# xiph/daala

Measured on AMD Instinct MI355X. Metric: 1080p all-intra transform blocks/s (filter+DCT+PVQ), higher is better.
Workload: dtype int32 (lifting DCT/filters) + f64 (PVQ search)

## Files before the change

daala_amd/csrc/od_occupancy.cuh:

```cuda
#pragma once
#ifndef ODHIP_SEARCH_OCC
# define ODHIP_SEARCH_OCC 0
#endif
#if ODHIP_SEARCH_OCC == 2
# define OD_SEARCH_OCC_ATTR __attribute__((amdgpu_waves_per_eu(2), amdgpu_num_vgpr(100)))
# define OD_SEARCH_VGPR_FLOOR() asm volatile("" ::: "v175")
#elif ODHIP_SEARCH_OCC == 3
# define OD_SEARCH_OCC_ATTR __attribute__((amdgpu_waves_per_eu(3), amdgpu_num_vgpr(68)))
# define OD_SEARCH_VGPR_FLOOR() asm volatile("" ::: "v128")
#else
# define OD_SEARCH_OCC_ATTR __attribute__((amdgpu_waves_per_eu(3)))
# define OD_DECIDE_OCC_ATTR
# define OD_SEARCH_VGPR_FLOOR() ((void)0)
#endif
#ifndef OD_DECIDE_OCC_ATTR
# define OD_DECIDE_OCC_ATTR OD_SEARCH_OCC_ATTR
#endif
#ifndef ODHIP_SEARCH_WAVES
# define ODHIP_SEARCH_WAVES 1
#endif
#ifndef ODHIP_PAIR_WAVES
# define ODHIP_PAIR_WAVES 8
#endif
#ifndef OD_PAIR_OCC_ATTR
# if ODHIP_SEARCH_OCC == 0
#  define OD_PAIR_OCC_ATTR __attribute__((amdgpu_waves_per_eu(4)))
# else
#  define OD_PAIR_OCC_ATTR OD_SEARCH_OCC_ATTR
# endif
#endif
```

daala_amd/csrc/pvq_refbands.hip:

```cpp
#include "../../include/daala_hip.h"
#include <math.h>
#include <stdio.h>
#include <stdlib.h>
#include <string.h>
#include "od_ctx.cuh"
#include "od_pvq_math.cuh"
#include "od_occupancy.cuh"
#include "od_krange.cuh"
#include "od_band_stage.cuh"
#include "gen/od_scan_tables.h"
#define OD_RSQ_TABLE_N 512
#define OD_RSQ_HUGE
#include "pvq_search.cuh"
#include "pvq_row.cuh"
#include "pvq_regs.cuh"
#include "pvq_lane.cuh"

namespace {

constexpr int kMaxJobs = 8;
constexpr int kMaxItems = kMaxJobs*ODHIP_MAX_BANDS;
constexpr int kSlots = ODHIP_PVQ_REF_SLOTS;
constexpr int kUncCap = 1 << 16;
constexpr double kDefaultMargin = 1e-9;
// ... 1246 lines not shown
      cos_out[band] = c;
      if (replays_out) replays_out[band] = replays;
    }
  }
  (void)n;
}

template <int E, int G>
__global__ __launch_bounds__(kWave) __attribute__((amdgpu_waves_per_eu(3, 3))) void k_refb_search_row(RItems it) {
  od_rsqrt_init(threadIdx.x);
  const int item = find_item(it, blockIdx.x);
  const RJob &jb = it.jobs[it.job[item]];
  const int lane = threadIdx.x;
  RowVector<E, G> v;
  v.row = lane/G;
  v.l = lane%G;
  v.force = it.perturb >> 1;
  const long nblocks = jb.nblocks;
  const long pos = (long)(blockIdx.x - it.wg_start[item])*(kWave/G) + v.row;
  const bool live = pos < nblocks;
  const long blk = jb.ids[(long)it.band[item]*nblocks + (live ? pos : nblocks - 1)];
  NoDecide nd;
  refb_loops(jb, it.band[item], blk, live && v.l == 0, live, it.lambda, v, nd);
}

template <int N>
struct RegVector {
  static constexpr int SH = N == 15 ? 1 : 0;
  int ax[N];
  unsigned sg;
  int y[N];
  double xx;
  double norm_1;
  double cxy;
  double cyy;
  __device__ __forceinline__ void load(const int16_t *src, bool pad) {
    const uint4 *p = reinterpret_cast<const uint4 *>(src - SH);
    sg = 0;
    uint32_t w[(N + SH)/2];
#pragma unroll
    for (int q = 0; q < (N + SH)/8; q++) {
      const uint4 t = p[q];
      w[4*q] = t.x;
      w[4*q + 1] = t.y;
      w[4*q + 2] = t.z;
      w[4*q + 3] = t.w;
    }
#pragma unroll
    for (int i = 0; i < N; i++) {
      const int t = (int16_t)(w[(i + SH) >> 1] >> (16*((i + SH) & 1)));
      ax[i] = abs(t);
      sg |= (unsigned)(t < 0) << i;
      y[i] = 0;
    }
    if (pad) {
      ax[N - 1] = 0;
      sg &= ~(1u << (N - 1));
    }
    od_regs_norm<N>(ax, &xx, &norm_1);
  }
  __device__ __forceinline__ double search(int n_true, int k, int prev_k, double g2, double lambda) {
    return od_pvq_search_regs<N>(ax, y, n_true, k, prev_k, g2, lambda, xx, norm_1, &cxy, &cyy);
  }
  __device__ __forceinline__ int moment() const {
    int m = 0;
#pragma unroll
    for (int i = 1; i < N; i++) m += i*y[i];
    return m;
  }
  __device__ __forceinline__ void store(int16_t *dst) {
    uint4 *p = reinterpret_cast<uint4 *>(dst - SH);
    int t[N + SH];
    if (SH) t[0] = 0;
#pragma unroll
    for (int i = 0; i < N; i++) t[i + SH] = (sg >> i) & 1 ? -y[i] : y[i];
#pragma unroll
    for (int q = 0; q < (N + SH)/8; q++) {
      p[q] = make_uint4(pack16(t[8*q], t[8*q + 1]), pack16(t[8*q + 2], t[8*q + 3]),
       pack16(t[8*q + 4], t[8*q + 5]), pack16(t[8*q + 6], t[8*q + 7]));
    }
  }
};

template <int NL>
struct PairVector {
  struct Pulses {
    const uint32_t *col;
    __device__ __forceinline__ int operator[](int e) const { return (int)(col[e*kPitch] >> 1 & 0x7fffu); }
  };
  uint32_t *pk;
  Pulses y;
  unsigned sg;
  int lane;
  int l;
  bool force_seq;
  LaneSearch st;
  __device__ __forceinline__ void init(uint32_t *columns, int lane_in, bool force) {
    pk = columns;
    y.col = columns + lane_in;
    lane = lane_in;
    l = lane_in & 1;
    force_seq = force;
  }
  __device__ __forceinline__ void load(const int16_t *src, bool pad) {
    static_assert(NL % 8 == 0, "whole 16-byte pieces");
    const uint4 *p = reinterpret_cast<const uint4 *>(src + l*NL);
    sg = 0;
#pragma unroll
    for (int q = 0; q < NL/8; q++) {
      const uint4 t = p[q];
      const uint32_t w[4] = {t.x, t.y, t.z, t.w};
#pragma unroll
      for (int e = 0; e < 8; e++) {
        const int j = 8*q + e;
        int v = (int16_t)(w[e >> 1] >> (16*(e & 1)));
        if (j == NL - 1 && pad && l == 1) v = 0;
        pk[j*kPitch + lane] = (uint32_t)abs(v) << 16;
        sg |= (unsigned)(v < 0) << j;
      }
    }
    od_lane_prepare<NL, 2>(st, pk, lane);
  }
  __device__ __forceinline__ double search(int n_true, int k, int prev_k, double g2, double lambda) {
    const bool fresh = !(prev_k > 0 && prev_k <= k);
    return od_lane_search<NL, 2, true>(st, pk, od_rsq_lds, lane, l, true, fresh, k, g2, lambda, force_seq,
     n_true != 2*NL);
  }
  __device__ __forceinline__ int moment() const {
    int m = 0;
#pragma unroll
    for (int e = 0; e < NL; e++) m += (l*NL + e)*y[e];
    return od_grp_add<2>(m);
  }
};

__device__ __forceinline__ int neg_interleave(int x, int ref) {
  if (x < ref) return -2*(x - ref) - 1;
  if (x < 2*ref) return 2*(x - ref);
  return x - 1;
}

__device__ unsigned char gRBandOf[OD_SCAN_LEN];

template <int N, class YGet>
__device__ __forceinline__ void refb_finish(const RItems &it, int job, const RJob &jb, int band, long blk,
 const odhip_pvq_refband &r, const RefBest &best, YGet yget);

template <int N, int PRICE>
__device__ __forceinline__ void refb_choose_band(const RItems &it, int job, const RJob &jb, int band,
 long blk, const double *given) {
  constexpr int SH = N == 15 ? 1 : 0;
  constexpr int NW = (N + SH)/2;
  const long bi = blk*jb.nb_bands + band;
  const odhip_pvq_refband r = jb.rec[bi];
  const ItemPtr ip = item_ptr(jb, band, blk);
  const double *rate = PRICE == 2 ? given : PRICE == 0 && jb.rate ? jb.rate + bi*(kSlots + 1) : nullptr;
  const double lambda = it.lambda;
  const int off = jb.off[band];
  double best_cost = r.dist0 + lambda*(rate ? rate[0] : 0.);
  bool close = false;
  int noref = jb.is_keyframe ? 1 : 0;
  int32_t best_qtheta = 0;
  int chosen = -1;
  int yslot = -1;
  int4 tails[kSlots];
  int dlo[kSlots];
  int dhi[kSlots];
#pragma unroll
  for (int idx = 0; idx < kSlots; idx++) {
    tails[idx] = make_int4(0, 0, 0, -1);
    dlo[idx] = 0;
    dhi[idx] = 0;
    if (idx < r.nitems) {
      tails[idx] = ip.tail[idx*ip.stride];
      const int4 res = ip.res[idx*ip.stride];
      dlo[idx] = res.z;
      dhi[idx] = res.w;
    }
  }
#pragma unroll
  for (int idx = 0; idx < kSlots; idx++) {
    if (idx >= r.nitems) continue;
    const int4 tail = tails[idx];
    if (!(tail.z & ODHIP_REFITEM_SEARCHED)) continue;
    double cost = __hiloint2double(dhi[idx], dlo[idx]);
    if (PRICE == 1) {
      const int4 hd = ip.head[idx*ip.stride];
      const bool with_ref = idx < r.ntheta;
      const int sum = (int)((unsigned)tail.z >> ODHIP_REFITEM_MOMENT_SHIFT);
      cost = cost + lambda*odq_pvq_rate_fast(sum, hd.w, N, hd.x, with_ref ? r.icgr : 0, with_ref ? hd.y : -1,
       with_ref ? hd.z : 0, jb.is_keyframe, jb.pli);
      const double d = cost - best_cost;
      if ((d < 0 ? -d : d) <= it.tol_scale*odq_rate_tol(cost, best_cost)) close = true;
    }
    else cost = cost + lambda*(rate ? rate[1 + idx] : 0.);
    if (idx < r.ntheta ? cost < best_cost : cost <= best_cost) {
      best_cost = cost;
      chosen = idx;
      yslot = tail.w;
      if (idx < r.ntheta) {
        best_qtheta = tail.y;
        noref = 0;
      }
      else noref = 1;
    }
  }
  RefBest best;
  best.best_cost = best_cost;
  best.chosen = chosen;
  best.yslot = yslot;
  best.noref = noref;
  best.qtheta = best_qtheta;
  best.gain = best.theta = best.ts = best.k = 0;
  best.close = PRICE == 1 && close;
  if (chosen >= 0) {
    const int4 head = ip.head[chosen*ip.stride];
    best.gain = head.x;
// ... 384 lines not shown
      dist = (1.4*(qcg - cg))*(qcg - cg) + (qcg*(double)cg)*dist_theta;
      dist *= s2;
      const double lts = __hiloint2double((int)cl.col[(kSlots + 7 + 2*gi)*cl.stride],
       (int)cl.col[(kSlots + 6 + 2*gi)*cl.stride]);
      dec.offer(idx - 1, true, i, j, ts, k, qtheta, dist, prate, lts, has, v);
    }
  }
  if (cl.nitems > cl.ntheta) {
    v.load(jb.x16 + blk*len + off, false);
    int prev_k = 0;
    int idx = cl.ntheta;
    while (idx < cl.nitems) {
      const uint32_t w = cl.col[idx*cl.stride];
      const int i = cl.gbn + (int)(w & 3u);
#ifdef ODHIP_EXPERIMENTS
      const int k = dec.abl & 8 ? 0 : (int)(w >> 2 & 0xffffu);
#else
      const int k = (int)(w >> 2 & 0xffffu);
#endif
      const int32_t qcg = odq_shl32(i, ODQ_CGAIN_SHIFT);
      double dist = (1.4*(qcg - cg))*(qcg - cg);
      dist *= s2;
      const bool skip = (dist > dist0 && k != 0) || k > ODHIP_PVQ_MAX_K;
      const bool others = __any(skip);
      if (!skip && others) continue;
      idx++;
      if (skip) continue;
      const double cos_dist = v.search(n, k, prev_k, (qcg*(double)cg)*s2, lambda);
      prev_k = k;
      const double prate = lean_rate_pulses<NR>(v.moment(), k);
      dist = (1.4*(qcg - cg))*(qcg - cg) + (qcg*(double)cg)*(2 - 2*cos_dist);
      dist *= s2;
      dec.offer(idx - 1, false, i, -1, 0, k, 0, dist, prate, 0., true, v);
    }
  }
}

constexpr int kPreWords = 6;
constexpr int kPrePacked = 1;

template <int NR, int G, class V, class D, bool PACKED = false, int WAVES = kSearchWaves>
__device__ __forceinline__ void refb_loops_lean_rows(const RJob &jb, int band, long blk,
 const odhip_pvq_refband &r, const CandList &cl, double lambda, V &v, D &dec, uint32_t *pre, int pre_stride) {
  const int off = jb.off[band];
  const int n = jb.off[band + 1] - off;
  const int len = jb.len;
  const double s2 = (1./256)*(1./256);
  const double t1 = 1./32768;
  const int32_t cg = r.cg;
  const double dist0 = r.dist0;
  const int32_t theta = r.theta;
  uint32_t skips = 0;
  for (int c = v.l; c < kSlots; c += G) {
    if (c < cl.ntheta) {
      const uint32_t w = cl.col[c*cl.stride];
      const int gi = (int)(w & 3u);
      const int k = (int)(w >> 2 & 0xffffu);
      const int i = cl.gb1 + gi;
      const int ts = (int)cl.col[(kSlots + gi)*cl.stride];
      const int j = (int)cl.col[(kSlots + 3 + gi)*cl.stride] + (int)(w >> 18);
      const int32_t qcg = odq_shl32(i, ODQ_CGAIN_SHIFT) + r.gain_offset;
      const int32_t qtheta = odq_pvq_compute_theta(j, ts);
      const int cosd = odq_pvq_cos(theta - qtheta);
      const double cosfix = 2 - (2.*cosd)*t1;
      double dist = (1.4*(qcg - cg))*(qcg - cg) + (qcg*(double)cg)*cosfix;
      dist *= s2;
      const bool skip = (dist > dist0 + 1.0*lambda && k != 0) || k > ODHIP_PVQ_MAX_K;
      if constexpr (PACKED) {
        skips |= (uint32_t)skip << c;
        pre[c*kPrePacked*pre_stride] = ((uint32_t)cosd & 0xffffu) | (uint32_t)odq_pvq_sin(qtheta) << 16;
      }
      else {
        const double sin_prod = ((odq_pvq_sin(theta)*t1)*odq_pvq_sin(qtheta))*t1;
        uint32_t *p = pre + c*kPreWords*pre_stride;
        p[0] = (uint32_t)qcg;
        p[pre_stride] = skip;
        p[2*pre_stride] = (uint32_t)__double2loint(cosfix);
        p[3*pre_stride] = (uint32_t)__double2hiint(cosfix);
        p[4*pre_stride] = (uint32_t)__double2loint(sin_prod);
        p[5*pre_stride] = (uint32_t)__double2hiint(sin_prod);
      }
    }
  }
  static_assert(!PACKED || (G == 2 && kSlots <= 32), "the two halves of a pair's skip mask");
  if constexpr (PACKED) skips = od_grp_or<2>(skips);
  if constexpr (WAVES == 1) __syncthreads();
  else {
    __builtin_amdgcn_fence(__ATOMIC_RELEASE, "wavefront");
    __builtin_amdgcn_wave_barrier();
    __builtin_amdgcn_fence(__ATOMIC_ACQUIRE, "wavefront");
  }
  if (cl.ntheta > 0) {
    v.load(jb.xr + blk*len + off, true);
    int prev_k = 0;
    bool has = false;
    double cos_dist = 0;
    double prate = 0;
    int idx = 0;
    while (idx < cl.ntheta) {
      const uint32_t w = cl.col[idx*cl.stride];
#ifdef ODHIP_EXPERIMENTS
      const int k = dec.abl & 8 ? 0 : (int)(w >> 2 & 0xffffu);
#else
      const int k = (int)(w >> 2 & 0xffffu);
#endif
      const uint32_t *p = pre + idx*(PACKED ? kPrePacked : kPreWords)*pre_stride;
      const bool skip = PACKED ? (skips >> idx & 1u) != 0 : p[pre_stride] != 0;
      const bool want = !skip && k != 0 && k != prev_k;
      const bool others = __any(!want);
      if (want && others) continue;
      idx++;
      if (skip) continue;
      const int gi = (int)(w & 3u);
      const int i = cl.gb1 + gi;
      const int ts = (int)cl.col[(kSlots + gi)*cl.stride];
      const int j = (int)cl.col[(kSlots + 3 + gi)*cl.stride] + (int)(w >> 18);
      int32_t qcg;
      double cosfix;
      double sin_prod;
      if constexpr (PACKED) {
        const uint32_t cs = p[0];
        qcg = odq_shl32(i, ODQ_CGAIN_SHIFT) + r.gain_offset;
        cosfix = 2 - (2.*(int16_t)(cs & 0xffffu))*t1;
        sin_prod = ((odq_pvq_sin(theta)*t1)*(int16_t)(cs >> 16))*t1;
      }
      else {
        qcg = (int32_t)p[0];
        cosfix = __hiloint2double((int)p[3*pre_stride], (int)p[2*pre_stride]);
        sin_prod = __hiloint2double((int)p[5*pre_stride], (int)p[4*pre_stride]);
      }
      if (k == 0) {
        cos_dist = 0;
        has = false;
        prate = 0;
      }
      else if (want) {
        cos_dist = v.search(n - 1, k, prev_k, ((qcg*(double)cg)*sin_prod)*s2, lambda);
        has = true;
        prate = lean_rate_pulses<NR>(v.moment(), k);
      }
      prev_k = k;
      const double dist_theta = cosfix + sin_prod*(2 - 2*cos_dist);
      double dist = (1.4*(qcg - cg))*(qcg - cg) + (qcg*(double)cg)*dist_theta;
      dist *= s2;
      const double lts = __hiloint2double((int)cl.col[(kSlots + 7 + 2*gi)*cl.stride],
       (int)cl.col[(kSlots + 6 + 2*gi)*cl.stride]);
      dec.offer(idx - 1, true, i, j, ts, k, 0, dist, prate, lts, has, v);
    }
  }
  if (cl.nitems > cl.ntheta) {
    v.load(jb.x16 + blk*len + off, false);
    int prev_k = 0;
    int idx = cl.ntheta;
    while (idx < cl.nitems) {
      const uint32_t w = cl.col[idx*cl.stride];
      const int i = cl.gbn + (int)(w & 3u);
#ifdef ODHIP_EXPERIMENTS
      const int k = dec.abl & 8 ? 0 : (int)(w >> 2 & 0xffffu);
#else
      const int k = (int)(w >> 2 & 0xffffu);
#endif
      const int32_t qcg = odq_shl32(i, ODQ_CGAIN_SHIFT);
      double dist = (1.4*(qcg - cg))*(qcg - cg);
      dist *= s2;
      const bool skip = (dist > dist0 && k != 0) || k > ODHIP_PVQ_MAX_K;
      const bool others = __any(skip);
      if (!skip && others) continue;
      idx++;
      if (skip) continue;
      const double cos_dist = v.search(n, k, prev_k, (qcg*(double)cg)*s2, lambda);
      prev_k = k;
      const double prate = lean_rate_pulses<NR>(v.moment(), k);
      dist = (1.4*(qcg - cg))*(qcg - cg) + (qcg*(double)cg)*(2 - 2*cos_dist);
      dist *= s2;
      dec.offer(idx - 1, false, i, -1, 0, k, 0, dist, prate, 0., true, v);
    }
  }
}

template <int NY>
struct LeanDecide {
  double best_cost;
  int chosen;
  bool close;
  int y[NY];
  unsigned sg;
  double lambda;
  double tol_scale;
  int icgr;
  int is_keyframe;
  int pli;
#ifdef ODHIP_EXPERIMENTS
  int abl = 0;
#endif
  __device__ __forceinline__ void init(const odhip_pvq_refband &r, const RJob &jb, double lam, double tol) {
    best_cost = r.dist0;
    chosen = -1;
    close = false;
    lambda = lam;
    tol_scale = tol;
    icgr = r.icgr;
    is_keyframe = jb.is_keyframe;
    pli = jb.pli;
    sg = 0;
#pragma unroll
    for (int i = 0; i < NY; i++) y[i] = 0;
  }
  template <class V>
  __device__ __forceinline__ void offer(int idx, bool with_ref, int i, int j, int ts, int k, int32_t qtheta,
   double dist, double prate, double lts, bool has, const V &v) {
    const double rate = odq_pvq_rate_join(prate, lts, i, with_ref ? icgr : 0, with_ref ? j : -1, is_keyframe,
     pli);
    const double cost = dist + lambda*rate;
    const double d = cost - best_cost;
    if ((d < 0 ? -d : d) <= tol_scale*odq_rate_tol(cost, best_cost)) close = true;
    if (with_ref ? cost < best_cost : cost <= best_cost) {
      best_cost = cost;
      chosen = idx;
      sg = v.sg;
#pragma unroll
      for (int e = 0; e < NY; e++) y[e] = has ? v.y[e] : 0;
    }
    (void)ts;
    (void)k;
    (void)qtheta;
  }
  __device__ __forceinline__ int signed_y(int e) const {
    return (sg >> e) & 1 ? -y[e] : y[e];
  }
};

template <int NY>
__device__ __forceinline__ RefBest lean_best(const LeanDecide<NY> &dec, const CandList &cl, int is_keyframe) {
  RefBest b;
  b.best_cost = dec.best_cost;
  b.chosen = dec.chosen;
  b.yslot = -1;
  b.noref = is_keyframe ? 1 : 0;
  b.qtheta = 0;
  b.gain = b.theta = b.ts = b.k = 0;
  b.close = dec.close;
  if (dec.chosen >= 0) {
    const uint32_t w = cl.col[dec.chosen*cl.stride];
    b.k = (int)(w >> 2 & 0xffffu);
    b.yslot = b.k > 0 ? 0 : -1;
    if (dec.chosen < cl.ntheta) {
      const int gi = (int)(w & 3u);
      b.noref = 0;
      b.gain = cl.gb1 + gi;
      b.ts = (int)cl.col[(kSlots + gi)*cl.stride];
      b.theta = (int)cl.col[(kSlots + 3 + gi)*cl.stride] + (int)(w >> 18);
      b.qtheta = odq_pvq_compute_theta(b.theta, b.ts);
    }
    else {
      b.noref = 1;
      b.gain = cl.gbn + (int)(w & 3u);
    }
  }
  return b;
}

template <int N>
__global__ __launch_bounds__(kSearchThreads) OD_SEARCH_OCC_ATTR void k_refb_lean_lane(RItems it) {
  constexpr int SH = N == 15 ? 1 : 0;
  __shared__ uint32_t s_list_w[kSearchWaves][kLeanWords*kWave];
  OD_SEARCH_VGPR_FLOOR();
  od_rsqrt_init(threadIdx.x);
  const int lane = threadIdx.x%kWave;
  const int wave = __builtin_amdgcn_readfirstlane(threadIdx.x/kWave);
// ... 138 lines not shown
    return;
  }
  const int m = r.m;
  const int s = r.s;
  scale = (int32_t)floor(.5 + (scale*(1./32768))*odq_pvq_sin(best.qtheta));
  const int16_t xm = (int16_t)floor(.5 + ((-s*odq_shr_round(g, gshift))*(1./32768))*odq_pvq_cos(best.qtheta));
  uint32_t rw[E/2];
#pragma unroll
  for (int q = 0; q < E/8; q++) {
    const uint4 r4 = reinterpret_cast<const uint4 *>(jb.r16 + blk*jb.len + off + l*E)[q];
    rw[4*q] = r4.x;
    rw[4*q + 1] = r4.y;
    rw[4*q + 2] = r4.z;
    rw[4*q + 3] = r4.w;
  }
  const int yprev = grp_from_prev<G>(wy[E - 1], l);
  int32_t l2r = 0;
  int32_t proj = 0;
#pragma unroll
  for (int e = 0; e < E; e++) {
    const int i = l*E + e;
    const int ri = (int16_t)(rw[e >> 1] >> (16*(e & 1)));
    const int ysrc = i < m ? wy[e] : (e == 0 ? yprev : wy[e > 0 ? e - 1 : 0]);
    const int16_t xi = i == m ? xm : (int16_t)odq_mult16_32_q16(ysrc, scale);
    l2r += odq_mult16_16(ri, ri);
    proj += odq_mult16_16(ri, xi);
  }
  l2r = grp_total<G>(l2r);
  proj = grp_total<G>(proj);
  int16_t proj_1;
  int outshift;
  householder_consts(l2r, proj, &proj_1, &outshift);
  if (writer) {
    ch[2] = make_int4(3, yslot, scale, qshift);
    ch[3] = make_int4(xm, m, proj_1, outshift);
  }
  (void)n;
}

template <int E, int G>
__global__ __launch_bounds__(kSearchThreads) OD_SEARCH_OCC_ATTR void k_refb_lean_row(RItems it) {
  constexpr int C = kWave/G;
  __shared__ uint32_t s_list_w[kSearchWaves][kLeanWords*C];
  __shared__ uint32_t s_pre_w[kSearchWaves][kSlots*kPreWords*C];
  OD_SEARCH_VGPR_FLOOR();
  od_rsqrt_init(threadIdx.x);
  const int wave = __builtin_amdgcn_readfirstlane(threadIdx.x/kWave);
  const int unit = blockIdx.x*kSearchWaves + wave;
  if (unit >= it.wg_start[it.nitems]) return;
  uint32_t *s_list = s_list_w[wave];
  uint32_t *s_pre = s_pre_w[wave];
  const int item = find_item(it, unit);
  const int job = it.job[item];
  const RJob &jb = it.jobs[job];
  const int band = it.band[item];
  const int lane = threadIdx.x%kWave;
  RowVector<E, G> v;
  v.row = lane/G;
  v.l = lane%G;
  v.force = it.perturb >> 1;
  const long nblocks = jb.nblocks;
  const long pos = (long)(unit - it.wg_start[item])*C + v.row;
  const bool live = pos < nblocks;
  const long blk = jb.ids[(long)band*nblocks + (live ? pos : nblocks - 1)];
  const odhip_pvq_refband r = jb.rec[blk*jb.nb_bands + band];
  const CandList cl = refb_build_list(jb, band, r, s_list + v.row, C, v.l == 0);
  LeanDecide<E> dec;
  dec.init(r, jb, it.lambda, it.tol_scale);
#ifdef ODHIP_EXPERIMENTS
  dec.abl = it.abl;
#endif
  refb_loops_lean_rows<G*E, G>(jb, band, blk, r, cl, it.lambda, v, dec, s_pre + v.row, C);
  refb_finish_row<E, G>(it, job, jb, band, blk, r, dec, lean_best(dec, cl, jb.is_keyframe), v.l, live);
#ifdef ODHIP_EXPERIMENTS
  if (live && v.l == 0) {
    if (v.pulses) atomicAdd(&gRowReplayStats[0], (unsigned long long)v.pulses);
    if (v.replays) atomicAdd(&gRowReplayStats[1], (unsigned long long)v.replays);
    if (v.rate_pulses) atomicAdd(&gRowReplayStats[2], (unsigned long long)v.rate_pulses);
    atomicAdd(&gRowReplayStats[3], 1ull);
  }
#endif
}

constexpr int kPairWaves = ODHIP_PAIR_WAVES;
constexpr int kPairThreads = kPairWaves*kWave;

template <int NL>
__global__ __launch_bounds__(kPairThreads) OD_PAIR_OCC_ATTR void k_refb_lean_pair(RItems it) {
  constexpr int G = 2;
  constexpr int C = kWave/G;
  static_assert(kRsqN == OD_RSQ_TABLE_N && kPitch == kWave, "od_lane_search on this unit's table and columns");
  __shared__ uint32_t s_list_w[kPairWaves][kLeanWords*C];
  __shared__ uint32_t s_pre_w[kPairWaves][kSlots*kPrePacked*C];
  __shared__ uint32_t s_pk_w[kPairWaves][NL*kPitch];
  OD_SEARCH_VGPR_FLOOR();
  od_rsqrt_init(threadIdx.x);
  const int wave = __builtin_amdgcn_readfirstlane(threadIdx.x/kWave);
  const int unit = blockIdx.x*kPairWaves + wave;
  if (unit >= it.wg_start[it.nitems]) return;
  uint32_t *s_list = s_list_w[wave];
  uint32_t *s_pre = s_pre_w[wave];
  const int item = find_item(it, unit);
  const int job = it.job[item];
  const RJob &jb = it.jobs[job];
  const int band = it.band[item];
  const int lane = threadIdx.x%kWave;
  const int row = lane/G;
  PairVector<NL> v;
  v.init(s_pk_w[wave], lane, (it.perturb >> 1) != 0);
  const long nblocks = jb.nblocks;
  const long pos = (long)(unit - it.wg_start[item])*C + row;
  const bool live = pos < nblocks;
  const long blk = jb.ids[(long)band*nblocks + (live ? pos : nblocks - 1)];
  const odhip_pvq_refband r = jb.rec[blk*jb.nb_bands + band];
  const CandList cl = refb_build_list(jb, band, r, s_list + row, C, v.l == 0);
  LeanDecide<NL> dec;
  dec.init(r, jb, it.lambda, it.tol_scale);
#ifdef ODHIP_EXPERIMENTS
  dec.abl = it.abl;
#endif
  refb_loops_lean_rows<G*NL, G, PairVector<NL>, LeanDecide<NL>, true, kPairWaves>(jb, band, blk, r, cl,
   it.lambda, v, dec, s_pre + row, C);
  refb_finish_row<NL, G>(it, job, jb, band, blk, r, dec, lean_best(dec, cl, jb.is_keyframe), v.l, live);
}

template <int N>
__global__ __launch_bounds__(kWave) void k_refb_choose_unc_list(RItems it, const Unc *list, int count) {
  const int i = blockIdx.x*kWave + threadIdx.x;
  if (i >= count) return;
  const Unc e = list[i];
  const RJob &jb = it.jobs[e.job];
  if (jb.off[e.band + 1] - jb.off[e.band] != N) return;
  refb_choose_band<N, 1>(it, e.job, jb, e.band, e.blk, nullptr);
}

template <int N, int PRICE>
__global__ __launch_bounds__(kWave) void k_refb_choose(RItems it) {
  const int item = find_item(it, blockIdx.x);
  const int job = it.job[item];
  const RJob &jb = it.jobs[job];
  const long blk = (long)(blockIdx.x - it.wg_start[item])*kWave + threadIdx.x;
  if (blk >= jb.nblocks) return;
  refb_choose_band<N, PRICE>(it, job, jb, it.band[item], blk, nullptr);
}

template <int N>
__global__ __launch_bounds__(kWave) void k_refb_choose_list(RItems it, const PUncR *list, int count) {
  const int i = blockIdx.x*kWave + threadIdx.x;
  if (i >= count) return;
  const PUncR *e = list + i;
  const RJob &jb = it.jobs[e->job];
  if (jb.off[e->band + 1] - jb.off[e->band] != N) return;
  refb_choose_band<N, 2>(it, e->job, jb, e->band, e->blk, e->rate);
}

__global__ __launch_bounds__(256) void k_refb_synth(RItems it) {
  const int item = find_item(it, blockIdx.x);
  const RJob &jb = it.jobs[it.job[item]];
  const int len = jb.len;
  const int cpb = len >> 3;
  const long t = (long)(blockIdx.x - it.wg_start[item])*256 + threadIdx.x;
  const long blk = t/cpb;
  if (blk >= jb.nblocks) return;
  const int c0 = (int)(t - blk*cpb) << 3;
  const long base = block_base(jb, blk);
  od_coeff *out = jb.dq + base;
  const int w = jb.w;
  const int band = gRBandOf[c0 ? c0 : 1];
  const int off = jb.off[band];
  const uint4 sc4 = *reinterpret_cast<const uint4 *>(gRScanPk + c0);
  const unsigned scw[4] = {sc4.x, sc4.y, sc4.z, sc4.w};
  long pos[8];
#pragma unroll
  for (int e = 0; e < 8; e++) {
    const unsigned pk = (scw[e >> 1] >> (16*(e & 1))) & 0xffffu;
    pos[e] = (long)(pk >> 8)*w + (pk & 255);
  }
  const int4 *ch = reinterpret_cast<const int4 *>(jb.choice + (blk*jb.nb_bands + band)*16);
  const int4 a = ch[2];
  const int mode = a.x;
  const int first = c0 == 0;
  if (first) out[0] = jb.coef[base];
  if (mode == 0) {
#pragma unroll
    for (int e = 0; e < 8; e++) if (!(first && e == 0)) out[pos[e]] = 0;
    return;
  }
  if (mode == 1 || mode == 4) {
#pragma unroll
    for (int e = 0; e < 8; e++) {
      if (first && e == 0) continue;
      const od_coeff rv = jb.ref[base + pos[e]];
      out[pos[e]] = mode == 4 ? -rv : rv;
    }
    return;
  }
  const int yslot = a.y;
  const int32_t scale = a.z;
  const int qshift = a.w;
  const uint4 q4 = *reinterpret_cast<const uint4 *>(jb.qm_inv + c0);
  const unsigned qw[4] = {q4.x, q4.y, q4.z, q4.w};
  unsigned yw[4] = {0, 0, 0, 0};
  int yprev = 0;
  if (yslot >= 0) {
// ... 202 lines not shown
  for (int i = 0; i < njobs; i++) {
    rc = fill_job(host[i], jobs[i], mode);
    if (rc) return rc;
    host[i].krange = st.counters.d.p + 2;
  }
  if (mode == kJobBands) {
    rc = st.sort.place(host, njobs, s);
    if (rc) return rc;
  }
  return st.tabs.upload(host, njobs, s);
}

int sort_weights(void) {
  static const int w = [] {
    int p = 4, c = 4, s = 8;
    const char *e = ODHIP_EXP_ENV("ODHIP_SORT_W");
    if (e) sscanf(e, "%d,%d,%d", &p, &c, &s);
    return (p & 255) | (c & 255) << 8 | (s & 255) << 16;
  }();
  return w;
}

void items_begin(RItems &it, const RefState &st, double lambda) {
  memset(&it, 0, sizeof(it));
  it.lambda = lambda;
  it.margin = st.margin;
  it.perturb = st.perturb;
  it.jobs = st.tabs.cur;
  it.unc_count = st.unc_count();
  it.unc = st.unc.p;
  it.pcount = st.pcount();
  it.plist = st.plist.p;
  it.tol_scale = st.tol_scale;
  it.sort_weights = sort_weights();
#ifdef ODHIP_EXPERIMENTS
  static const int abl = [] {
    const char *e = getenv("ODHIP_REFB_ABL");
    return e ? atoi(e) : 0;
  }();
  it.abl = abl;
#endif
}

enum RefStage {
  kStageRecords = 0,
  kStageLanePriced = 1,
  kStageDecided = 2
};

void launch_prep(const RefState &st, const RJob *host, int njobs, double lambda, RefStage stage, hipStream_t s) {
  RItems pi;
  const auto prep = [&](void (*kernel)(RItems), int size, long per_wg) {
    items_begin(pi, st, lambda);
    pi.fuse = stage;
    if (size) items_add_size(pi, host, njobs, size, per_wg, 1);
    else for (int j = 0; j < njobs; j++) items_add(pi, j, 0, (host[j].nblocks + per_wg - 1)/per_wg);
    if (pi.nitems) kernel<<<pi.wg_start[pi.nitems], kWave, 0, s>>>(pi);
  };
#ifdef ODHIP_EXPERIMENTS
  static const bool split = getenv("ODHIP_REFB_PREP_SPLIT") != nullptr;
  if (split) {
    prep(k_refb_prep_lane<15>, 0, kWave);
    prep(k_refb_prep_lane<8>, 8, kWave);
  }
  else
#endif
  prep(k_refb_prep_corner, 0, kWave);
  prep(k_refb_prep_row<8, 4>, 32, 16);
  prep(k_refb_prep_row<8, 16>, 128, 4);
}

int sort_blocks(RefState &st, const RJob *host, int njobs, hipStream_t s) {
  return st.sort.run(host, st.tabs.cur, njobs, s);
}

struct RefSearch {
  int size;
  int on;
  int per_wg;
  bool row;
};
constexpr RefSearch kRefSearches[4] = {{128, 0, 4, true}, {32, 1, 16, true}, {15, 2, kWave, false},
 {8, 2, kWave, false}};
constexpr int kPairBands = kWave/2;

bool pair_search(const RefSearch &r, RefStage stage) {
  static const bool row32 = ODHIP_EXP_ENV("ODHIP_REFB_ROW32") != nullptr;
  return r.size == 32 && stage == kStageDecided && !row32;
}

void launch_search(RefState &st, RItems &it, const RefSearch &r, RefStage stage, hipStream_t s) {
  if (stage == kStageDecided) items_heavy_first(it);
  const int wgs = it.wg_start[it.nitems];
  const int groups = (wgs + kSearchWaves - 1)/kSearchWaves;
  const auto regs = [&](auto priced) {
    for_band_size(r.size, [&](auto size) {
      constexpr int N = decltype(size)::value;
      if constexpr (N <= 15) k_refb_search_regs<N, decltype(priced)::value><<<wgs, kWave, 0, s>>>(it);
    });
  };
  const auto launch = [&] {
    if (pair_search(r, stage)) k_refb_lean_pair<16><<<(wgs + kPairWaves - 1)/kPairWaves, kPairThreads, 0, s>>>(it);
    else if (r.row) {
      for_band_size(r.size, [&](auto size) {
        constexpr int N = decltype(size)::value;
        if constexpr (N >= 32) {
          if (stage == kStageDecided) k_refb_lean_row<8, N/8><<<groups, kSearchThreads, 0, s>>>(it);
          else k_refb_search_row<8, N/8><<<wgs, kWave, 0, s>>>(it);
        }
      });
    }
    else if (stage == kStageDecided) {
      for_band_size(r.size, [&](auto size) {
        constexpr int N = decltype(size)::value;
        if constexpr (N <= 15) k_refb_lean_lane<N><<<groups, kSearchThreads, 0, s>>>(it);
      });
    }
    else if (stage == kStageLanePriced) regs(std::true_type());
    else regs(std::false_type());
  };
  if (r.size == 128) st.prof.around(s, launch);
  else launch();
}

int launch_searches(RefState &st, const RJob *host, int njobs, double lambda, RefStage stage, hipStream_t s) {
  const bool lane_only = stage != kStageDecided && ODHIP_EXP_ENV("ODHIP_PVQ_REF_LANE") != nullptr;
  hipStream_t side[2] = {s, s};
  if (st.streams.fork(s, side) != ODHIP_SUCCESS) return ODHIP_EFAULT;
  const hipStream_t streams[3] = {s, side[0], side[1]};
  RItems it;
  for (const RefSearch &r : kRefSearches) {
    items_begin(it, st, lambda);
    if (r.row && !lane_only && odhip_env_force_seq()) it.perturb |= 2;
    items_add_size(it, host, njobs, r.size, lane_only ? kWave : pair_search(r, stage) ? kPairBands : r.per_wg);
    if (it.nitems && !lane_only) launch_search(st, it, r, stage, streams[r.on]);
#ifdef ODHIP_EXPERIMENTS
    if (it.nitems && lane_only) {
      k_refb_search<<<it.wg_start[it.nitems], kWave, (size_t)2*r.size*kWave*sizeof(unsigned short), streams[r.on]>>>(it);
    }
#endif
  }
  if (st.streams.join(s, side) != ODHIP_SUCCESS) return ODHIP_EFAULT;
  return ODHIP_SUCCESS;
}

int ref_bands(const odhip_pvq_refjob *jobs, int njobs, double pvq_norm_lambda, odhip_stream stream, RefStage stage) {
  hipStream_t s = (hipStream_t)stream;
  REF_STATE_OR_RETURN(st);
  RJob host[kMaxJobs];
  int rc = stage_jobs(st, jobs, njobs, kJobBands, host, s);
  if (rc) return rc;
  ODHIP_TRY(hipMemsetAsync(st.unc_count(), 0, (stage != kStageRecords ? 2 : 1)*sizeof(unsigned), s));
  st.lean = stage == kStageDecided;
  RItems it;
  items_begin(it, st, pvq_norm_lambda);
  items_add_size(it, host, njobs, 0, kWave);
  if (!it.nitems) return ODHIP_SUCCESS;
  launch_prep(st, host, njobs, pvq_norm_lambda, stage, s);
  if (stage != kStageDecided) k_refb_cands<<<it.wg_start[it.nitems], kWave, 0, s>>>(it);
  rc = sort_blocks(st, host, njobs, s);
  if (rc) return rc;
  rc = launch_searches(st, host, njobs, pvq_norm_lambda, stage, s);
  if (rc) return rc;
  if (stage == kStageDecided) {
    rc = st.unc_posted.post(st.unc_count(), s);
    if (!rc) rc = st.priced.post(st.pcount(), s);
    if (rc) return rc;
  }
  return odhip_check_launch();
}

void rerun_listed(const RefState &st, const Unc *d_list, unsigned n, double lambda, hipStream_t s) {
  k_refb_cands_list<<<(n + kWave - 1)/kWave, kWave, 0, s>>>(st.tabs.cur, d_list, (int)n);
  k_refb_search_list<<<n, kWave, (size_t)2*128*kWave*sizeof(unsigned short), s>>>(st.tabs.cur, d_list, (int)n,
   lambda);
}

void decide_listed(RefState &st, const Unc *d_list, unsigned n, double lambda, hipStream_t s) {
  RItems it;
  items_begin(it, st, lambda);
  const unsigned grid = (n + kWave - 1)/kWave;
  for (const int size : kBandSizes) {
    for_band_size(size, [&](auto N) {
      k_refb_choose_unc_list<decltype(N)::value><<<grid, kWave, 0, s>>>(it, d_list, (int)n);
    });
  }
  (void)st.priced.post(st.pcount(), s);
}

enum RefSelect {
  kSelectSynth,
  kSelectChoice,
  kSelectPriced,
  kSelectPricedRest
};

int ref_select(const odhip_pvq_refjob *jobs, int njobs, double pvq_norm_lambda, hipStream_t s, RefSelect sel) {
  const bool synth = sel == kSelectSynth;
  const bool price = sel == kSelectPriced || sel == kSelectPricedRest;
  REF_STATE_OR_RETURN(st);
  RJob host[kMaxJobs];
  int rc = stage_jobs(st, jobs, njobs, synth ? kJobSynth : kJobChoice, host, s);
  if (rc) return rc;
  for (int j = 0; synth && j < njobs; j++) {
    if (host[j].bs >= 3) {
      const size_t bytes = sizeof(od_coeff)*(size_t)host[j].nplanes*host[j].w*host[j].h;
      if (host[j].is_keyframe) ODHIP_TRY(hipMemsetAsync(host[j].dq, 0, bytes, s));
      else ODHIP_TRY(hipMemcpyAsync(host[j].dq, host[j].ref, bytes, hipMemcpyDeviceToDevice, s));
    }
  }
  if (sel == kSelectPriced) ODHIP_TRY(hipMemsetAsync(st.pcount(), 0, sizeof(unsigned), s));
  RItems it;
  const auto choose = [&](int n, auto priced) {
    for_band_size(n, [&](auto N) {
      k_refb_choose<decltype(N)::value, decltype(priced)::value><<<it.wg_start[it.nitems], kWave, 0, s>>>(it);
    });
  };
// ... 234 lines not shown
```

Measured before the change: 1.232 billion.

## Search 128-coefficient bands with lane groups in the decided PVQ stage

Generalizes the pair-lane lean search kernel into a GroupVector kernel, where S lanes share one band and each lane holds NL coefficients. In the decided stage, 128-coefficient bands now run through this kernel with four lanes per band (32 coefficients each) instead of the row kernel that packs 4 bands per workgroup. The goal is to fit 16 bands into each wave and cut the per-band serial work, at the cost of more LDS per wave, 64-bit sign masks, and different occupancy and wave-count settings.

```diff
diff --git a/daala_amd/csrc/od_occupancy.cuh b/daala_amd/csrc/od_occupancy.cuh
--- a/daala_amd/csrc/od_occupancy.cuh
+++ b/daala_amd/csrc/od_occupancy.cuh
@@ -22,10 +22,29 @@
 #ifndef ODHIP_PAIR_WAVES
 # define ODHIP_PAIR_WAVES 8
 #endif
-#ifndef OD_PAIR_OCC_ATTR
+#ifndef ODHIP_PAIR_OCC
+# define ODHIP_PAIR_OCC 4
+#endif
+#ifndef ODHIP_GROUP128_LANES
+# define ODHIP_GROUP128_LANES 4
+#endif
+#ifndef ODHIP_GROUP128_WAVES
+# define ODHIP_GROUP128_WAVES 4
+#endif
+#ifndef ODHIP_GROUP128_OCC
+# define ODHIP_GROUP128_OCC 3
+#endif
+#ifndef ODHIP_GROUP128_PAIR_WAVES
+# define ODHIP_GROUP128_PAIR_WAVES 6
+#endif
+#ifndef ODHIP_GROUP128_PAIR_OCC
+# define ODHIP_GROUP128_PAIR_OCC 2
+#endif
+#ifndef OD_GROUP_OCC_ATTR
 # if ODHIP_SEARCH_OCC == 0
-#  define OD_PAIR_OCC_ATTR __attribute__((amdgpu_waves_per_eu(4)))
+#  define OD_GROUP_OCC_ATTR(nl, s) __attribute__((amdgpu_waves_per_eu( \
+    (nl)*(s) == 32 ? ODHIP_PAIR_OCC : (s) == 4 ? ODHIP_GROUP128_OCC : ODHIP_GROUP128_PAIR_OCC)))
 # else
-#  define OD_PAIR_OCC_ATTR OD_SEARCH_OCC_ATTR
+#  define OD_GROUP_OCC_ATTR(nl, s) OD_SEARCH_OCC_ATTR
 # endif
 #endif
diff --git a/daala_amd/csrc/pvq_refbands.hip b/daala_amd/csrc/pvq_refbands.hip
--- a/daala_amd/csrc/pvq_refbands.hip
+++ b/daala_amd/csrc/pvq_refbands.hip
@@ -1352,15 +1352,22 @@
   }
 };
 
-template <int NL>
-struct PairVector {
+template <int NY>
+struct LeanSigns {
+  using type = std::conditional_t<(NY > 32), unsigned long long, unsigned>;
+};
+
+template <int NL, int S>
+struct GroupVector {
+  static_assert(S == 2 || S == 4, "a pair or a quad per band");
   struct Pulses {
     const uint32_t *col;
     __device__ __forceinline__ int operator[](int e) const { return (int)(col[e*kPitch] >> 1 & 0x7fffu); }
   };
+  using Signs = typename LeanSigns<NL>::type;
   uint32_t *pk;
   Pulses y;
-  unsigned sg;
+  Signs sg;
   int lane;
   int l;
   bool force_seq;
@@ -1369,7 +1376,7 @@
     pk = columns;
     y.col = columns + lane_in;
     lane = lane_in;
-    l = lane_in & 1;
+    l = lane_in & (S - 1);
     force_seq = force;
   }
   __device__ __forceinline__ void load(const int16_t *src, bool pad) {
@@ -1384,25 +1391,27 @@
       for (int e = 0; e < 8; e++) {
         const int j = 8*q + e;
         int v = (int16_t)(w[e >> 1] >> (16*(e & 1)));
-        if (j == NL - 1 && pad && l == 1) v = 0;
+        if (j == NL - 1 && pad && l == S - 1) v = 0;
         pk[j*kPitch + lane] = (uint32_t)abs(v) << 16;
-        sg |= (unsigned)(v < 0) << j;
+        sg |= (Signs)(v < 0) << j;
       }
     }
-    od_lane_prepare<NL, 2>(st, pk, lane);
+    od_lane_prepare<NL, S>(st, pk, lane);
   }
   __device__ __forceinline__ double search(int n_true, int k, int prev_k, double g2, double lambda) {
     const bool fresh = !(prev_k > 0 && prev_k <= k);
-    return od_lane_search<NL, 2, true>(st, pk, od_rsq_lds, lane, l, true, fresh, k, g2, lambda, force_seq,
-     n_true != 2*NL);
+    return od_lane_search<NL, S, true>(st, pk, od_rsq_lds, lane, l, true, fresh, k, g2, lambda, force_seq,
+     n_true != S*NL);
   }
   __device__ __forceinline__ int moment() const {
     int m = 0;
 #pragma unroll
     for (int e = 0; e < NL; e++) m += (l*NL + e)*y[e];
-    return od_grp_add<2>(m);
+    return od_grp_add<S>(m);
   }
 };
+template <int NL>
+using PairVector = GroupVector<NL, 2>;
 
 __device__ __forceinline__ int neg_interleave(int x, int ref) {
   if (x < ref) return -2*(x - ref) - 1;
@@ -1953,8 +1962,8 @@
       }
     }
   }
-  static_assert(!PACKED || (G == 2 && kSlots <= 32), "the two halves of a pair's skip mask");
-  if constexpr (PACKED) skips = od_grp_or<2>(skips);
+  static_assert(!PACKED || ((G == 2 || G == 4) && kSlots <= 32), "the parts of a group's skip mask");
+  if constexpr (PACKED) skips = od_grp_or<G>(skips);
   if constexpr (WAVES == 1) __syncthreads();
   else {
     __builtin_amdgcn_fence(__ATOMIC_RELEASE, "wavefront");
@@ -2055,7 +2064,7 @@
   int chosen;
   bool close;
   int y[NY];
-  unsigned sg;
+  typename LeanSigns<NY>::type sg;
   double lambda;
   double tol_scale;
   int icgr;
@@ -2360,21 +2369,25 @@
 #endif
 }
 
-constexpr int kPairWaves = ODHIP_PAIR_WAVES;
-constexpr int kPairThreads = kPairWaves*kWave;
-
-template <int NL>
-__global__ __launch_bounds__(kPairThreads) OD_PAIR_OCC_ATTR void k_refb_lean_pair(RItems it) {
-  constexpr int G = 2;
+constexpr int kGroup128Lanes = ODHIP_GROUP128_LANES;
+static_assert(kGroup128Lanes == 4 || kGroup128Lanes == 2, "a quad or a pair per 128-coefficient band");
+
+template <int NL, int S>
+constexpr int kGroupWaves = NL*S == 32 ? ODHIP_PAIR_WAVES : S == 4 ? ODHIP_GROUP128_WAVES : ODHIP_GROUP128_PAIR_WAVES;
+
+template <int NL, int S>
+__global__ __launch_bounds__((kGroupWaves<NL, S>*kWave)) OD_GROUP_OCC_ATTR(NL, S) void k_refb_lean_pair(RItems it) {
+  constexpr int G = S;
+  constexpr int WAVES = kGroupWaves<NL, S>;
   constexpr int C = kWave/G;
   static_assert(kRsqN == OD_RSQ_TABLE_N && kPitch == kWave, "od_lane_search on this unit's table and columns");
-  __shared__ uint32_t s_list_w[kPairWaves][kLeanWords*C];
-  __shared__ uint32_t s_pre_w[kPairWaves][kSlots*kPrePacked*C];
-  __shared__ uint32_t s_pk_w[kPairWaves][NL*kPitch];
+  __shared__ uint32_t s_list_w[WAVES][kLeanWords*C];
+  __shared__ uint32_t s_pre_w[WAVES][kSlots*kPrePacked*C];
+  __shared__ uint32_t s_pk_w[WAVES][NL*kPitch];
   OD_SEARCH_VGPR_FLOOR();
   od_rsqrt_init(threadIdx.x);
   const int wave = __builtin_amdgcn_readfirstlane(threadIdx.x/kWave);
-  const int unit = blockIdx.x*kPairWaves + wave;
+  const int unit = blockIdx.x*WAVES + wave;
   if (unit >= it.wg_start[it.nitems]) return;
   uint32_t *s_list = s_list_w[wave];
   uint32_t *s_pre = s_pre_w[wave];
@@ -2384,7 +2397,7 @@
   const int band = it.band[item];
   const int lane = threadIdx.x%kWave;
   const int row = lane/G;
-  PairVector<NL> v;
+  GroupVector<NL, S> v;
   v.init(s_pk_w[wave], lane, (it.perturb >> 1) != 0);
   const long nblocks = jb.nblocks;
   const long pos = (long)(unit - it.wg_start[item])*C + row;
@@ -2397,7 +2410,7 @@
 #ifdef ODHIP_EXPERIMENTS
   dec.abl = it.abl;
 #endif
-  refb_loops_lean_rows<G*NL, G, PairVector<NL>, LeanDecide<NL>, true, kPairWaves>(jb, band, blk, r, cl,
+  refb_loops_lean_rows<G*NL, G, GroupVector<NL, S>, LeanDecide<NL>, true, WAVES>(jb, band, blk, r, cl,
    it.lambda, v, dec, s_pre + row, C);
   refb_finish_row<NL, G>(it, job, jb, band, blk, r, dec, lean_best(dec, cl, jb.is_keyframe), v.l, live);
 }
@@ -2766,11 +2779,26 @@
 };
 constexpr RefSearch kRefSearches[4] = {{128, 0, 4, true}, {32, 1, 16, true}, {15, 2, kWave, false},
  {8, 2, kWave, false}};
-constexpr int kPairBands = kWave/2;
-
-bool pair_search(const RefSearch &r, RefStage stage) {
-  static const bool row32 = ODHIP_EXP_ENV("ODHIP_REFB_ROW32") != nullptr;
-  return r.size == 32 && stage == kStageDecided && !row32;
+
+int group_lanes(const RefSearch &r, RefStage stage) {
+  if (stage != kStageDecided) return 0;
+  if (r.size == 32) {
+    static const bool row32 = ODHIP_EXP_ENV("ODHIP_REFB_ROW32") != nullptr;
+    return row32 ? 0 : 2;
+  }
+  if (r.size == 128) {
+#ifdef ODHIP_EXPERIMENTS
+    static const int lanes = [] {
+      const char *e = ODHIP_EXP_ENV("ODHIP_REFB_GROUP128");
+      const int v = e ? atoi(e) : 0;
+      return v == 4 || v == 2 ? v : 0;
+    }();
+    return lanes;
+#else
+    return kGroup128Lanes;
+#endif
+  }
+  return 0;
 }
 
 void launch_search(RefState &st, RItems &it, const RefSearch &r, RefStage stage, hipStream_t s) {
@@ -2783,8 +2811,21 @@
       if constexpr (N <= 15) k_refb_search_regs<N, decltype(priced)::value><<<wgs, kWave, 0, s>>>(it);
     });
   };
+  const int lanes = group_lanes(r, stage);
+  const auto group = [&](auto nl, auto lanes_c) {
+    constexpr int NL = decltype(nl)::value;
+    constexpr int S = decltype(lanes_c)::value;
+    constexpr int W = kGroupWaves<NL, S>;
+    k_refb_lean_pair<NL, S><<<(wgs + W - 1)/W, W*kWave, 0, s>>>(it);
+  };
   const auto launch = [&] {
-    if (pair_search(r, stage)) k_refb_lean_pair<16><<<(wgs + kPairWaves - 1)/kPairWaves, kPairThreads, 0, s>>>(it);
+    if (lanes && r.size == 32) group(std::integral_constant<int, 16>(), std::integral_constant<int, 2>());
+#if defined(ODHIP_EXPERIMENTS) || ODHIP_GROUP128_LANES == 4
+    else if (lanes == 4) group(std::integral_constant<int, 32>(), std::integral_constant<int, 4>());
+#endif
+#if defined(ODHIP_EXPERIMENTS) || ODHIP_GROUP128_LANES == 2
+    else if (lanes == 2) group(std::integral_constant<int, 64>(), std::integral_constant<int, 2>());
+#endif
     else if (r.row) {
       for_band_size(r.size, [&](auto size) {
         constexpr int N = decltype(size)::value;
@@ -2816,7 +2857,8 @@
   for (const RefSearch &r : kRefSearches) {
     items_begin(it, st, lambda);
     if (r.row && !lane_only && odhip_env_force_seq()) it.perturb |= 2;
-    items_add_size(it, host, njobs, r.size, lane_only ? kWave : pair_search(r, stage) ? kPairBands : r.per_wg);
+    const int lanes = group_lanes(r, stage);
+    items_add_size(it, host, njobs, r.size, lane_only ? kWave : lanes ? kWave/lanes : r.per_wg);
     if (it.nitems && !lane_only) launch_search(st, it, r, stage, streams[r.on]);
 #ifdef ODHIP_EXPERIMENTS
     if (it.nitems && lane_only) {
```

Result: faster. 1.309 billion, median of 6 (+6.2%).
